# mako443/Text2Pos-CVPR2022

Hardware: AMD Instinct MI355X
Metric: cells+queries encoded/sec and top-k retrieval QPS, 256-pt cells, 12k-cell DB (higher is better)
Workload: dtype f16x3 (fp32 operands split hi+lo into fp16, 3 f16 MFMAs, fp32 accumulate; fp32-class error) for the encoders / f64 MFMA for the ranking

## Files before the change

include/t2p.h:

```cpp
#ifndef T2P_H
#define T2P_H
#include <stddef.h>
#include <stdint.h>

#ifdef __cplusplus
extern "C" {
#endif

#define T2P_ABI_VERSION 32
#define T2P_DEFAULT_CHUNK_OBJECTS 65000
#define T2P_MAX_CHUNK_OBJECTS 65535
#define T2P_TUNING_MASK 0xD
#define T2P_E_ARG (-1)
#define T2P_E_WORKSPACE (-2)
#define T2P_E_UNSUPPORTED (-3)

typedef void* t2p_stream_t;

int t2p_abi_version(void);
const char* t2p_last_error(void);

typedef struct t2p_cell_weights {
    const float* sa_w1[3];
    const float* sa_b1[3];
// ... 177 lines not shown
    const float* w_ih;
    const float* w_hh;
    const float* bias;
    const void* w_hh_x3;
    float w_hh_scale;
} t2p_text_weights;

size_t t2p_encode_text_workspace_bytes(int64_t batch, int32_t vocab, int32_t embed_dim);

int t2p_encode_text(const int32_t* tokens, const int32_t* lengths, int64_t batch, int32_t max_len, int32_t vocab,
                    int32_t embed_dim, const t2p_text_weights* w, float* out_raw, float* out, void* workspace,
                    size_t workspace_bytes, t2p_stream_t stream);

#define T2P_SIM_TOPK_MAX_K 1024
#define T2P_SIM_TOPK_REG_K 16
#define T2P_SIM_TOPK_TILE_BYTES ((size_t)256 << 20)
size_t t2p_sim_topk_workspace_bytes(int64_t nq, int64_t nc, int32_t k);
int t2p_sim_topk(const float* queries, const float* cells, int64_t nq, int64_t nc, int32_t dim, int32_t k,
                 int64_t index_offset, int64_t* out_idx, double* out_score, void* workspace, size_t workspace_bytes,
                 t2p_stream_t stream);
int t2p_sim_topk_grouped(const float* queries, const float* cells, const int32_t* query_group, const int32_t* cell_group,
                         int64_t nq, int64_t nc, int32_t dim, int32_t k, int64_t index_offset, int64_t* out_idx,
                         double* out_score, void* workspace, size_t workspace_bytes, t2p_stream_t stream);

void t2p_profile_enable(int on);
int t2p_profile_report(char* buf, size_t buf_bytes);
void t2p_profile_repeat(const char* scope, int32_t reps);

int t2p_lstm_train_forward(const float* gate_table, const float* w_hh_k, const int32_t* tokens, const int32_t* lengths,
                           int64_t batch, int32_t max_len, int32_t embed_dim, int32_t reverse, float* gates, float* cs, float* hs,
// ... 44 lines not shown
int t2p_sample_group(const float* xyz, int64_t n_obj, int32_t n_pts, const float* radius_host ,
                     uint8_t* const* fps_idx , uint8_t* const* nbr , uint8_t* const* cnt ,
                     t2p_stream_t stream);
int t2p_group_rows(const float* xyz, int64_t n_obj, int32_t n_pts, const float* radius_host , int32_t self_loops,
                   uint8_t* const* fps_idx , uint16_t* const* rows , uint16_t* const* n_rows ,
                   t2p_stream_t stream);
int t2p_group_rows_shared(const float* xyz, int64_t n_obj, int32_t n_pts, const float* radius_host , int32_t self_loops,
                          int32_t share_mask, uint8_t* const* fps_idx , uint16_t* const* rows ,
                          uint16_t* const* n_rows , t2p_stream_t stream);
int t2p_group_rows_built(const float* xyz, const float* rgb, int64_t n_obj, int32_t n_pts, const float* radius_host ,
                         int32_t self_loops, int32_t share_mask, uint8_t* const* fps_idx , uint16_t* const* rows ,
                         uint16_t* const* n_rows , t2p_stream_t stream);
int t2p_group_rows_pruned(const float* xyz, const float* rgb, int64_t n_obj, int32_t n_pts, const float* radius_host ,
                          int32_t self_loops, int32_t share_mask, uint8_t* const* fps_idx , uint16_t* const* rows ,
                          uint16_t* const* n_rows , t2p_stream_t stream);
int t2p_edge_counts(const uint16_t* rows, const uint16_t* n_rows, const int32_t* first_obj, int64_t n_obj, int32_t n_dense,
                    int32_t n_cent, int32_t self_loops, int32_t* counts, t2p_stream_t stream);
int t2p_edge_expand(const uint16_t* rows, const uint16_t* n_rows, const int32_t* first_obj, const int32_t* cent_ptr, int64_t n_obj,
                    int32_t n_dense, int32_t n_cent, int32_t self_loops, int32_t* src, int32_t* dst, t2p_stream_t stream);
int t2p_dedup_rows(const float* xyz, const float* rgb, int64_t n_obj, int32_t n_pts, uint16_t* rows, uint16_t* n_rows,
                   t2p_stream_t stream);
int t2p_knn(const float* x, int32_t dim, const int32_t* seg_ptr, int32_t n_seg, int32_t max_seg_rows, int32_t k,
            int32_t* out_idx, t2p_stream_t stream);
int t2p_gemm(const float* a, int32_t lda, const float* w, const float* bias, float* c, int32_t ldc, int32_t c0,
             int64_t m, int32_t k, int32_t n, int32_t relu, t2p_stream_t stream);
int t2p_gemm_residual(const float* a, int32_t lda, const float* w, const float* bias, float* c, int32_t ldc, int32_t c0,
                      int64_t m, int32_t k, int32_t n, int32_t relu, const float* resid, int32_t ldr, t2p_stream_t stream);
int t2p_gemm_x3(const float* a, int32_t lda, const void* wx, float scale, const float* bias, float* c, int32_t ldc, int32_t c0,
                int64_t m, int32_t k, int32_t n, int32_t relu, const float* resid, int32_t ldr, uint32_t* amax_in,
                t2p_stream_t stream);
// ... 15 lines not shown
```

profiles/topk_sweep.py:

```python
import argparse
import json
import os
import sys

import numpy as np
import torch

ROOT = os.path.dirname(os.path.dirname(os.path.abspath(__file__)))
sys.path.insert(0, ROOT)
import text2pos_amd as t2p
from text2pos_amd import ops


def timed(fn, steps, warmup, calls):
    ms = []
    for i in range(warmup + steps):
        e0, e1 = torch.cuda.Event(enable_timing=True), torch.cuda.Event(enable_timing=True)
        e0.record()
        for _ in range(calls):
            fn()
        e1.record()
        e1.synchronize()
        if i >= warmup:
            ms.append(e0.elapsed_time(e1) / calls)
# ... 6 lines not shown
        e0.record()
        for _ in range(calls):
            fn()
        e1.record()
        e1.synchronize()
        return e0.elapsed_time(e1) / calls
    a_ms, b_ms = [], []
    for i in range(warmup + steps):
        ta, tb = window(fn_a), window(fn_b)
        if i >= warmup:
            a_ms.append(ta)
            b_ms.append(tb)
    return float(np.median(a_ms)), float(np.median(b_ms)), [b / a for a, b in zip(a_ms, b_ms)]


def main():
    ap = argparse.ArgumentParser()
    ap.add_argument("--shapes", default="1000x12000,1250x100000")
    ap.add_argument("--ks", default="10,16,17,32,100,256,1024")
    ap.add_argument("--dim", type=int, default=256)
    ap.add_argument("--steps", type=int, default=9)
    ap.add_argument("--warmup", type=int, default=3)
    ap.add_argument("--calls", type=int, default=0, help="calls per timed window (0: 20 for the small shape, 3 above 10^8 scores)")
    ap.add_argument("--groups", type=int, default=0, help="also time the group-restricted call with this many group ids")
    ap.add_argument("--skip-torch", action="store_true", help="do not time torch's float64 GEMM + topk")
    a = ap.parse_args()
    assert torch.cuda.is_available(), "topk_sweep needs cuda:0: there is no CPU path to time"
    dev = torch.device("cuda:0")
    for shape in a.shapes.split(","):
        nq, nc = (int(x) for x in shape.split("x"))
        g = torch.Generator().manual_seed(nq * 31 + nc)
        c = torch.nn.functional.normalize(torch.randn(nc, a.dim, generator=g), dim=-1).to(dev)
        q = torch.nn.functional.normalize(torch.randn(nq, a.dim, generator=g), dim=-1).to(dev)
        calls = a.calls or (20 if nq * nc <= 10 ** 8 else 3)
        cd, qd = c.double(), q.double()
        if a.groups:
            cg = torch.randint(0, a.groups, (nc,), generator=g).to(torch.int32).to(dev)
            qg = torch.randint(0, a.groups, (nq,), generator=g).to(torch.int32).to(dev)
        for k in (int(x) for x in a.ks.split(",")):
            med, lo, hi = timed(lambda: t2p.retrieve_topk(c, q, k), a.steps, a.warmup, calls)
            t_med, t_lo, t_hi = (0.0, 0.0, 0.0) if a.skip_torch else timed(lambda: (qd @ cd.T).topk(k), a.steps, a.warmup, calls)
            grouped = {}
            if a.groups:
                u_ms, g_ms, ratios = timed_pairs(lambda: t2p.retrieve_topk(c, q, k),
# ... 33 lines not shown
```

text2pos-cvpr2022_amd/_lib.py:

```python
import ctypes as C
import os

import torch

_HERE = os.path.dirname(os.path.abspath(__file__))
LIB_PATH = os.environ.get("T2P_LIB") or os.path.join(_HERE, "libt2p_hip.so")
ABI_VERSION = 32

c_float_p = C.POINTER(C.c_float)
c_void = C.c_void_p


class CellWeights(C.Structure):
    _names = (["sa_w1", "sa_b1", "sa_w2", "sa_b2"], ["ga_w1", "ga_b1", "ga_w2", "ga_b2", "lin1_w", "lin1_b", "lin2_w",
              "lin2_b", "pn_w", "pn_b", "col_w1", "col_b1", "col_w2", "col_b2", "pos_w1", "pos_b1", "pos_w2", "pos_b2",
              "merge_w", "merge_b", "g_wp", "g_bp", "g_wq", "g_w2", "g_b2", "lin_w1", "lin_b1", "lin_w2", "lin_b2"])
    _fields_ = ([(n, c_void * 3) for n in _names[0]] + [(n, c_void) for n in _names[1]] +
                [("sa_w2_x3", c_void * 3), ("ga_w2_x3", c_void), ("sa_b2_x3", c_void * 3), ("sa_w2_scale", C.c_float * 3),
                 ("lin1_x3", c_void), ("lin2_x3", c_void), ("merge_x3", c_void), ("pn_x3", c_void), ("g_wp_x3", c_void),
                 ("g_wq_x3", c_void), ("lin1_scale", C.c_float), ("lin2_scale", C.c_float), ("merge_scale", C.c_float),
                 ("pn_scale", C.c_float), ("g_wp_scale", C.c_float), ("g_wq_scale", C.c_float),
                 ("sa_w1_x3", c_void * 3), ("ga_w1_x3", c_void),
                 ("class_embedding", c_void), ("color_embedding", c_void),
                 ("ga_w1_l1", C.c_float), ("ga_b1_absmax", C.c_float), ("sa_wp_l1", C.c_float * 3),
# ... 104 lines not shown
                                     C.c_int64, c_void, c_void, c_void, c_void, c_void, c_void, c_void]),
    "t2p_colsum": (C.c_int, [c_void, C.c_int64, C.c_int32, c_void, c_void]),
    "t2p_profile_enable": (None, [C.c_int]),
    "t2p_profile_report": (C.c_int, [C.c_char_p, C.c_size_t]),
    "t2p_profile_repeat": (None, [C.c_char_p, C.c_int32]),
    "t2p_sample_group": (C.c_int, [c_void, C.c_int64, C.c_int32, c_float_p, C.POINTER(c_void), C.POINTER(c_void),
                                   C.POINTER(c_void), c_void]),
    "t2p_group_rows": (C.c_int, [c_void, C.c_int64, C.c_int32, c_float_p, C.c_int32, C.POINTER(c_void), C.POINTER(c_void),
                                 C.POINTER(c_void), c_void]),
    "t2p_group_rows_shared": (C.c_int, [c_void, C.c_int64, C.c_int32, c_float_p, C.c_int32, C.c_int32, C.POINTER(c_void),
                                        C.POINTER(c_void), C.POINTER(c_void), c_void]),
    "t2p_group_rows_built": (C.c_int, [c_void, c_void, C.c_int64, C.c_int32, c_float_p, C.c_int32, C.c_int32, C.POINTER(c_void),
                                       C.POINTER(c_void), C.POINTER(c_void), c_void]),
    "t2p_group_rows_pruned": (C.c_int, [c_void, c_void, C.c_int64, C.c_int32, c_float_p, C.c_int32, C.c_int32, C.POINTER(c_void),
                                        C.POINTER(c_void), C.POINTER(c_void), c_void]),
    "t2p_edge_counts": (C.c_int, [c_void, c_void, c_void, C.c_int64, C.c_int32, C.c_int32, C.c_int32, c_void, c_void]),
    "t2p_edge_expand": (C.c_int, [c_void, c_void, c_void, c_void, C.c_int64, C.c_int32, C.c_int32, C.c_int32, c_void, c_void, c_void]),
    "t2p_dedup_rows": (C.c_int, [c_void, c_void, C.c_int64, C.c_int32, c_void, c_void, c_void]),
    "t2p_knn": (C.c_int, [c_void, C.c_int32, c_void, C.c_int32, C.c_int32, C.c_int32, c_void, c_void]),
    "t2p_gemm": (C.c_int, [c_void, C.c_int32, c_void, c_void, c_void, C.c_int32, C.c_int32, C.c_int64, C.c_int32,
                           C.c_int32, C.c_int32, c_void]),
    "t2p_rownorm": (C.c_int, [c_void, C.c_int64, C.c_int32, c_void, c_void]),
    "t2p_gemm_residual": (C.c_int, [c_void, C.c_int32, c_void, c_void, c_void, C.c_int32, C.c_int32, C.c_int64, C.c_int32,
                                    C.c_int32, C.c_int32, c_void, C.c_int32, c_void]),
    "t2p_gemm_x3": (C.c_int, [c_void, C.c_int32, c_void, C.c_float, c_void, c_void, C.c_int32, C.c_int32, C.c_int64, C.c_int32,
                              C.c_int32, C.c_int32, c_void, C.c_int32, c_void, c_void]),
    "t2p_gemm_skinny": (C.c_int, [c_void, C.c_int32, c_void, c_void, C.c_int32, C.c_int64, C.c_int32, C.c_int32, c_void]),
    "t2p_linear_wgrad_workspace_bytes": (C.c_size_t, [C.c_int64, C.c_int32, C.c_int32]),
    "t2p_linear_wgrad_f32": (C.c_int, [c_void, C.c_int32, c_void, C.c_int32, c_void, C.c_int32, c_void, C.c_int64, C.c_int32,
                                       C.c_int32, c_void, C.c_size_t, c_void]),
# ... 34 lines not shown
```

text2pos-cvpr2022_amd/csrc/api.hip:

```cpp
#include <stdarg.h>
#include <stdlib.h>
#include <math.h>
#include <string.h>

#include <mutex>
#include <set>
#include <utility>

#include "../../include/t2p.h"
#include "t2p_common.h"

namespace t2p {

static thread_local char g_err[512] = "";

void set_error(const char* fmt, ...) {
    va_list ap;
    va_start(ap, fmt);
    vsnprintf(g_err, sizeof(g_err), fmt, ap);
    va_end(ap);
}

int num_cus() {
    static int cached = 0;
// ... 374 lines not shown
    return launch_sim_topk(queries, cells, nq, nc, dim, k, index_offset, out_idx, out_score, workspace, workspace_bytes,
                           (hipStream_t)stream);
}

int t2p_sim_topk_grouped(const float* queries, const float* cells, const int32_t* query_group, const int32_t* cell_group,
                         int64_t nq, int64_t nc, int32_t dim, int32_t k, int64_t index_offset, int64_t* out_idx,
                         double* out_score, void* workspace, size_t workspace_bytes, t2p_stream_t stream) {
    T2P_CHECK_ARG(nq >= 0 && nc >= 0, "sim_topk_grouped: negative size");
    T2P_CHECK_ARG((queries != nullptr || nq == 0) && (cells != nullptr || nc == 0) &&
                      ((out_idx != nullptr && out_score != nullptr) || nq == 0 || k < 1),
                  "sim_topk_grouped: NULL argument");
    return launch_sim_topk_grouped(queries, cells, query_group, cell_group, nq, nc, dim, k, index_offset, out_idx, out_score,
                                   workspace, workspace_bytes, (hipStream_t)stream);
}

int t2p_edge_counts(const uint16_t* rows, const uint16_t* n_rows, const int32_t* first_obj, int64_t n_obj, int32_t n_dense,
                    int32_t n_cent, int32_t self_loops, int32_t* counts, t2p_stream_t stream) {
    T2P_CHECK_ARG(n_obj >= 0 && (n_obj == 0 || (rows && n_rows && first_obj && counts)), "edge_counts: NULL argument");
    return launch_edge_counts(rows, n_rows, first_obj, n_obj, n_dense, n_cent, self_loops, counts, (hipStream_t)stream);
}

int t2p_edge_expand(const uint16_t* rows, const uint16_t* n_rows, const int32_t* first_obj, const int32_t* cent_ptr, int64_t n_obj,
                    int32_t n_dense, int32_t n_cent, int32_t self_loops, int32_t* src, int32_t* dst, t2p_stream_t stream) {
    T2P_CHECK_ARG(n_obj >= 0 && (n_obj == 0 || (rows && n_rows && first_obj && cent_ptr)), "edge_expand: NULL argument");
    return launch_edge_expand(rows, n_rows, first_obj, cent_ptr, n_obj, n_dense, n_cent, self_loops, src, dst, (hipStream_t)stream);
}

int t2p_pack_objects(const float* raw_xyz, const float* raw_rgb, const int32_t* obj_ptr, const int32_t* sample_idx,
                     const float* rot_cos_sin, int64_t n_obj, int32_t n_pts, float* xyz, float* rgb, float* center, float* mean_rgb,
                     t2p_stream_t stream) {
// ... 105 lines not shown
```

text2pos-cvpr2022_amd/csrc/sim_topk.hip:

```cpp
#include "t2p_common.h"

namespace t2p {
namespace {

constexpr int KREG = 16;
constexpr int KCAP = KREG;
constexpr int KMAX = 1024;
constexpr int QB = 128;
constexpr int CB = 32;
typedef double f64x2 __attribute__((ext_vector_type(2)));
typedef int i32x4 __attribute__((ext_vector_type(4)));

struct Cand {
    double s;
    int i;
};
__device__ __forceinline__ bool better(double s, int i, double s2, int i2) { return s > s2 || (s == s2 && i < i2); }

__device__ __forceinline__ int d_row(int lane, int reg) { return (lane >> 4) + 4 * reg; }

__device__ __forceinline__ int tile_pos(int c) { return (c & ~15) | ((c & 3) << 2) | ((c >> 2) & 3); }

template <int DIM, bool GROUPED, class Epi>
__device__ __forceinline__ void sim_product_loop(const float* __restrict__ Q, const float* __restrict__ Cm, int64_t nq,
// ... 430 lines not shown
}

template <int DIM>
void launch_scores(dim3 grid, hipStream_t st, const float* Q, const float* Cm, const int32_t* qg, const int32_t* cg, int64_t nq,
                   int64_t nc, int cps, double* S, int64_t ld_s) {
    if (qg) hipLaunchKernelGGL((k_sim_scores<DIM, true>), grid, dim3(256), 0, st, Q, Cm, qg, cg, nq, nc, cps, S, ld_s);
    else hipLaunchKernelGGL((k_sim_scores<DIM, false>), grid, dim3(256), 0, st, Q, Cm, qg, cg, nq, nc, cps, S, ld_s);
}
template <int DIM>
void launch_partial(dim3 grid, hipStream_t st, const float* Q, const float* Cm, const int32_t* qg, const int32_t* cg, int64_t nq,
                    int64_t nc, int cps, double* ps, int* pi, int sp) {
    if (qg) hipLaunchKernelGGL((k_sim_partial<DIM, true>), grid, dim3(256), 0, st, Q, Cm, qg, cg, nq, nc, cps, ps, pi, sp);
    else hipLaunchKernelGGL((k_sim_partial<DIM, false>), grid, dim3(256), 0, st, Q, Cm, qg, cg, nq, nc, cps, ps, pi, sp);
}

int sim_topk_impl(const float* Q, const float* Cm, const int32_t* qg, const int32_t* cg, int64_t nq, int64_t nc, int dim, int k,
                  int64_t c_index_offset, int64_t* out_idx, double* out_score, void* ws, size_t ws_bytes, hipStream_t st);

}

size_t sim_topk_workspace_bytes(int64_t nq, int64_t nc, int k) {
    if (k > KREG) return (size_t)score_chunk(nq, nc) * score_ld(nc) * sizeof(double) + 256;
    const int sp = pick_splits(nq, nc);
    return (size_t)nq * sp * 4 * KCAP * (sizeof(double) + sizeof(int)) + 256;
}

int launch_sim_topk(const float* Q, const float* Cm, int64_t nq, int64_t nc, int dim, int k, int64_t c_index_offset,
                    int64_t* out_idx, double* out_score, void* ws, size_t ws_bytes, hipStream_t st) {
    return sim_topk_impl(Q, Cm, nullptr, nullptr, nq, nc, dim, k, c_index_offset, out_idx, out_score, ws, ws_bytes, st);
}

int launch_sim_topk_grouped(const float* Q, const float* Cm, const int32_t* query_group, const int32_t* cell_group, int64_t nq,
                            int64_t nc, int dim, int k, int64_t c_index_offset, int64_t* out_idx, double* out_score, void* ws,
                            size_t ws_bytes, hipStream_t st) {
    T2P_CHECK_ARG((query_group != nullptr || nq == 0) && (cell_group != nullptr || nc == 0), "sim_topk_grouped: NULL group array");
    return sim_topk_impl(Q, Cm, query_group, cell_group, nq, nc, dim, k, c_index_offset, out_idx, out_score, ws, ws_bytes, st);
}
// ... 2 lines not shown
int sim_topk_impl(const float* Q, const float* Cm, const int32_t* qg, const int32_t* cg, int64_t nq, int64_t nc, int dim, int k,
                  int64_t c_index_offset, int64_t* out_idx, double* out_score, void* ws, size_t ws_bytes, hipStream_t st) {
    T2P_CHECK_ARG(k >= 1 && k <= KMAX, "sim_topk: k=%d outside [1,%d]", k, KMAX);
    T2P_CHECK_ARG(dim == 256 || dim == 128 || dim == 384, "sim_topk: dim=%d not instantiated (128, 256, 384)", dim);
    T2P_CHECK_ARG(nc < 0x7fffffff, "sim_topk: nc too large");
    T2P_CHECK_ARG((((uintptr_t)Q) & 15) == 0 && (((uintptr_t)Cm) & 15) == 0, "sim_topk: Q and C must be 16-byte aligned");
    T2P_CHECK_ARG(k <= KREG || score_chunk(1, nc) > 0,
                  "sim_topk: k=%d > %d keeps one query's float64 scores (8 B x nc=%lld) in a workspace tile of at most %zu B: nc too large",
                  k, KREG, (long long)nc, kScoreTileBytes);
    if (nq == 0) return 0;
    const size_t need = sim_topk_workspace_bytes(nq, nc, k);
    if (ws_bytes < need || ws == nullptr) {
        set_error("sim_topk: workspace %zu B < required %zu B", ws_bytes, need);
        return T2P_E_WORKSPACE;
    }
    if (k > KREG) {
        T2P_CHECK_ARG((((uintptr_t)ws) & 15) == 0, "sim_topk: workspace must be 16-byte aligned");
        const int64_t chunk = score_chunk(nq, nc), ld_s = score_ld(nc);
        double* S = (double*)ws;
        for (int64_t qa = 0; qa < nq; qa += chunk) {
            const int64_t n = (nq - qa) < chunk ? (nq - qa) : chunk;
            if (nc > 0) {
                const int sp = pick_splits(n, nc);
                int cps = (int)((nc + sp - 1) / sp);
                cps = ((cps + CB - 1) / CB) * CB;
                const dim3 grid((unsigned)((n + QB - 1) / QB), (unsigned)sp);
                ProfScope ps_("sim_scores", st);
                const int32_t* qga = qg ? qg + qa : nullptr;
                if (dim == 256) launch_scores<256>(grid, st, Q + qa * dim, Cm, qga, cg, n, nc, cps, S, ld_s);
                else if (dim == 384) launch_scores<384>(grid, st, Q + qa * dim, Cm, qga, cg, n, nc, cps, S, ld_s);
                else launch_scores<128>(grid, st, Q + qa * dim, Cm, qga, cg, n, nc, cps, S, ld_s);
// ... 33 lines not shown
```

text2pos-cvpr2022_amd/csrc/small_kernels.hip:

```cpp
#include "t2p_common.h"

namespace t2p {
namespace {

__global__ __launch_bounds__(256) void k_rownorm(const float* __restrict__ in, int ld_in, int64_t n_rows, int dim,
                                                 float* __restrict__ out, int ld_out, int col0) {
    const int lane = threadIdx.x & 63;
    int64_t row = (int64_t)blockIdx.x * 4 + (threadIdx.x >> 6);
    if (row >= n_rows) return;
    const float* x = in + row * ld_in;
    float ss = 0.f;
    for (int i = lane; i < dim; i += 64) ss = fmaf(x[i], x[i], ss);
#pragma unroll
    for (int off = 32; off >= 1; off >>= 1) ss += __shfl_xor(ss, off, 64);
    float nrm = sqrtf(ss);
    float den = nrm > 1e-12f ? nrm : 1e-12f;
    float* y = out + row * ld_out + col0;
    for (int i = lane; i < dim; i += 64) y[i] = x[i] / den;
}

__global__ __launch_bounds__(256) void k_gather_rownorm(const float* __restrict__ table, const int32_t* __restrict__ idx,
                                                        int64_t n_rows, int dim, float* __restrict__ out, int ld_out,
                                                        int col0) {
    const int lane = threadIdx.x & 63;
// ... 147 lines not shown
        for (int off = 32; off >= 1; off >>= 1) v += __shfl_xor(v, off, 64);
        if ((tid & 63) == 0) ss[tid >> 6][r] = v;
    }
    __syncthreads();
#pragma unroll
    for (int j = 0; j < 2; j++) {
        const int c = tid + 256 * j;
        if (c >= D) break;
#pragma unroll
        for (int r = 0; r < kMlp3Rows; r++) {
            if (row0 + r >= n_rows) break;
            const float nrm = sqrtf((ss[0][r] + ss[1][r]) + (ss[2][r] + ss[3][r]));
            out[(row0 + r) * ld_out + col0 + c] = o[j][r] / (nrm > 1e-12f ? nrm : 1e-12f);
        }
    }
}

__device__ __forceinline__ uint64_t pack_mix64(uint64_t x) {
    x += 0x9E3779B97F4A7C15ull;
    x = (x ^ (x >> 30)) * 0xBF58476D1CE4E5B9ull;
    x = (x ^ (x >> 27)) * 0x94D049BB133111EBull;
    return x ^ (x >> 31);
}

__device__ __forceinline__ void aten_column_sums(const float* __restrict__ pts, int n_pts, int lane, float& sx, float& sy, float& sz) {
    float part = 0.f;
    if (lane < 12) {
        const int c = lane >> 2, k = lane & 3;
        const int size_ilp = n_pts >> 2;
        float acc[4] = {0.f, 0.f, 0.f, 0.f};
// ... 340 lines not shown
}

int launch_segmax(const float* in, int dim, const int32_t* seg_ptr, int n_seg, float* out, int mean, hipStream_t st) {
    if (n_seg == 0) return 0;
    ProfScope ps_("segpool", st);
    hipLaunchKernelGGL(k_segpool, dim3(n_seg), dim3(256), 0, st, in, dim, seg_ptr, n_seg, out, mean);
    T2P_CHECK_LAUNCH("segpool");
    return 0;
}

int launch_mlp3_norm(const float* in3, int64_t n_rows, const float* w1, const float* b1, const float* w2,
                     const float* b2, int D, float* out, int ld_out, int col0, hipStream_t st) {
    T2P_CHECK_ARG(D % 64 == 0 && D <= 512, "mlp3_norm: D=%d must be a multiple of 64, <= 512", D);
    if (n_rows == 0) return 0;
    ProfScope ps_("mlp3_norm", st);
    if (n_rows >= 16384)
        hipLaunchKernelGGL(k_mlp3_norm<32>, dim3((unsigned)((n_rows + 31) / 32)), dim3(256), 0, st, in3, n_rows, w1, b1, w2, b2, D, out, ld_out,
                           col0);
    else
        hipLaunchKernelGGL(k_mlp3_norm<8>, dim3((unsigned)((n_rows + 7) / 8)), dim3(256), 0, st, in3, n_rows, w1, b1, w2, b2, D, out, ld_out,
                           col0);
    T2P_CHECK_LAUNCH("mlp3_norm");
    return 0;
}

int launch_pack_objects(const float* raw_xyz, const float* raw_rgb, const int32_t* obj_ptr, const int32_t* sample_idx,
                        const float* rot, int64_t n_obj, int n_pts, float* xyz, float* rgb, float* center, float* mean_rgb,
                        hipStream_t st) {
    T2P_CHECK_ARG(n_pts <= 1024, "pack_objects: n_pts=%d > 1024 (the sampled points of an object are staged in LDS)", n_pts);
    if (n_obj == 0) return 0;
    ProfScope ps_("pack_objects", st);
    hipLaunchKernelGGL(k_pack_objects, dim3((unsigned)((n_obj + 3) / 4)), dim3(256), (size_t)4 * n_pts * 3 * sizeof(float), st, raw_xyz,
                       raw_rgb, obj_ptr, sample_idx, rot, n_obj, n_pts, xyz, rgb, center, mean_rgb);
    T2P_CHECK_LAUNCH("pack_objects");
// ... 88 lines not shown
```

text2pos-cvpr2022_amd/csrc/t2p_common.h:

```cpp
#pragma once
#include <hip/hip_runtime.h>
#include <stdint.h>
#include <stdio.h>

namespace t2p {

void set_error(const char* fmt, ...);

#define T2P_E_ARG (-1)
#define T2P_E_WORKSPACE (-2)
#define T2P_E_UNSUPPORTED (-3)

#define T2P_CHECK_ARG(cond, ...)                  \
    do {                                          \
        if (!(cond)) {                            \
            ::t2p::set_error(__VA_ARGS__);        \
            return T2P_E_ARG;                     \
        }                                         \
    } while (0)

#define T2P_CHECK_LAUNCH(name)                                                   \
    do {                                                                         \
        hipError_t e__ = hipGetLastError();                                      \
        if (e__ != hipSuccess) {                                                 \
// ... 253 lines not shown
    const float* pos_src;
    int ld_pos, pos_col0;
    const float* feat_src;
    const float* w1;
    const float* b1;
    int n_dense, n_cent;
    int64_t n_obj;
    int32_t* prefix_ws;
    int32_t* bounds_ws;
    int balanced;
    uint32_t* amax_out;
    int out_rows;
};
int launch_ws_sa(int H, int C, const SaParams& p, hipStream_t st);
int launch_sa_balance(const SaParams& p, int tile_rows, int n_wg, hipStream_t st);
constexpr int kSaTailCode = 64;
bool sa_rows_selected(int H, int C, const SaParams& p);
int launch_sa_rows(int H, int C, const SaParams& p, hipStream_t st);
int sa_rows_launch_shape(int64_t n_obj, int* tile_rows, int* n_wg);
bool sa_points_selected(int H, int C, const SaParams& p);
int launch_sa_points(int H, int C, const SaParams& p, hipStream_t st);
int sa_points_launch_shape(int64_t n_obj, int* tile_rows, int* n_wg);
bool sa3_selected(int H, int C, const SaParams& p);
int launch_sa3(const SaParams& p, hipStream_t st);
int sa3_launch_shape(int64_t n_obj, int* tile_rows, int* n_wg);
inline bool sa_shares_tail_rows(int l, int H, int C, const SaParams& p, int n_pts, int tuning) {
    return l == 1 && n_pts == 256 && !(tuning & 4) && p.n_dense == 128 && p.n_cent == 64 && sa_rows_selected(H, C, p);
}
int launch_sa_balance_levels(const SaParams p[3], const int H[3], const int C[3], hipStream_t st);

// ... 47 lines not shown
```

text2pos-cvpr2022_amd/csrc/ws_sa.hip:

```cpp
#include <type_traits>

#include "t2p_common.h"

namespace t2p {
namespace {

constexpr int kSub = 512;
constexpr int NT = 512;

template <int K, int N, int WN, int RT, bool X3>
struct SaCfg {
    static constexpr int WM = 8 / WN;
    static constexpr int NTW = N / (32 * WN);
    static constexpr int TR = WM * RT * 32;
    static constexpr int KS = K / 2;
    static constexpr int S16 = K / 16;
    static constexpr int WPLANES = X3 ? 2 : 1;
    static constexpr int WSTEPS = X3 ? S16 : KS;
    static constexpr int LD = X3 ? K + 8 : K + 4;
    static constexpr int PLANE = TR * LD;
    static constexpr int ACC_INTS = 8192 + N;
    static constexpr int F4_PER_ROW = K / 4;
    static constexpr int ITERS = TR * F4_PER_ROW / NT;
    static_assert(TR * F4_PER_ROW % NT == 0, "staging must divide evenly over the workgroup");
    static_assert(ITERS == 2 || ITERS == 4, "metadata vector is 4 or 8 bytes");
    static constexpr size_t lds_bytes() {
        return (size_t)2 * PLANE * 4 + (size_t)2 * ACC_INTS * 4 + 2 * TR + kSub * 2 + kSub * 4;
    }
};

__device__ __forceinline__ void balance_body(const uint16_t* __restrict__ n_rows, int n, int tile_rows, int n_wg,
                                             int32_t* __restrict__ prefix, int32_t* __restrict__ bounds) {
    __shared__ int part[1024];
    const int tid = threadIdx.x;
    const int per = (n + 1023) / 1024;
    const int lo = tid * per, hi = (lo + per) < n ? (lo + per) : n;
    int s = 0;
    for (int i = lo; i < hi; i++) s += ((int)n_rows[i] + tile_rows - 1) / tile_rows;
    part[tid] = s;
    __syncthreads();
    for (int off = 1; off < 1024; off <<= 1) {
        int v = tid >= off ? part[tid - off] : 0;
        __syncthreads();
        part[tid] += v;
        __syncthreads();
    }
    int run = part[tid] - s;
    for (int i = lo; i < hi; i++) {
        prefix[i] = run;
        run += ((int)n_rows[i] + tile_rows - 1) / tile_rows;
    }
    if (tid == 1023) prefix[n] = part[1023];
    __syncthreads();
    const int total = part[1023];
    for (int b = tid; b <= n_wg; b += 1024) {
        const long long target = ((long long)b * total) / n_wg;
        int l = 0, r = n;
        while (l < r) {
            const int m = (l + r) >> 1;
            if (prefix[m] < target) l = m + 1; else r = m;
        }
        bounds[b] = b == n_wg ? n : l;
    }
}

__global__ __launch_bounds__(1024) void k_balance(const uint16_t* __restrict__ n_rows, int n, int tile_rows, int n_wg,
                                                  int32_t* __restrict__ prefix, int32_t* __restrict__ bounds) {
    balance_body(n_rows, n, tile_rows, n_wg, prefix, bounds);
}

struct BalanceJobs {
    const uint16_t* n_rows[3];
    int32_t* prefix[3];
    int32_t* bounds[3];
    int tile_rows[3], n_wg[3];
    int n;
};
__global__ __launch_bounds__(1024) void k_balance_levels(BalanceJobs j) {
    const int l = blockIdx.x;
    balance_body(j.n_rows[l], j.n, j.tile_rows[l], j.n_wg[l], j.prefix[l], j.bounds[l]);
}

struct BatchIt {
    int gi;
    int r0;
    int n;
};

template <int K, int N, int WN, int RT, bool X3>
__global__ __launch_bounds__(NT, 2) void k_sa_stream(SaParams p) {
    using C = SaCfg<K, N, WN, RT, X3>;
    using TileT = std::conditional_t<X3, _Float16, float>;
    using WReg = std::conditional_t<X3, half8, float>;
// ... 246 lines not shown
            if (valid(it_d)) write_tile((t + 1) & 1, meta_d);
            fix_meta(it_m, meta_m);
            meta_d = meta_m;
            it_c = it_d;
            it_d = it_m;
            it_m = advance(it_m);
            __syncthreads();
        }
        if (flush_g >= 0) flush(flush_g, flush_buf);
    }
    if constexpr (X3) guard_publish_exact(p.amax_out, gmax);
}

}

int launch_sa_balance(const SaParams& p, int tile_rows, int n_wg, hipStream_t st) {
    ProfScope ps_("sa_balance", st);
    hipLaunchKernelGGL(k_balance, dim3(1), dim3(1024), 0, st, p.n_rows, (int)p.n_obj, tile_rows, n_wg, p.prefix_ws,
                       p.bounds_ws);
    T2P_CHECK_LAUNCH("sa_balance");
    return 0;
}

namespace {

#define SA_STREAM_CASES(X) X(32, 64, 2, 2) X(128, 128, 4, 1) X(256, 256, 8, 1)

int sa_stream_shape(int H, int Cout, bool x3, int64_t n_obj, int* tile_rows, int* n_wg) {
    int n = num_cus();
    if (n > 1024) n = 1024;
    if (n > n_obj) n = (int)n_obj;
    *n_wg = n;
#define SA_CASE(K_, N_, WN_, RT_)                           \
    if (H == K_ && Cout == N_) {                            \
        *tile_rows = SaCfg<K_, N_, WN_, RT_, false>::TR;    \
        return 0;                                           \
// ... 69 lines not shown
}

}

int launch_sa_balance_levels(const SaParams p[3], const int H[3], const int C[3], hipStream_t st) {
    if (p[0].n_obj <= 0) return 0;
    BalanceJobs j;
    j.n = (int)p[0].n_obj;
    for (int l = 0; l < 3; l++) {
        j.n_rows[l] = p[l].n_rows;
        j.prefix[l] = p[l].prefix_ws;
        j.bounds[l] = p[l].bounds_ws;
        T2P_TRY(sa_launch_shape(H[l], C[l], p[l], p[l].n_obj, &j.tile_rows[l], &j.n_wg[l]));
    }
    ProfScope ps_("sa_balance", st);
    hipLaunchKernelGGL(k_balance_levels, dim3(3), dim3(1024), 0, st, j);
    T2P_CHECK_LAUNCH("sa_balance");
    return 0;
}

int launch_ws_sa(int H, int Cout, const SaParams& p, hipStream_t st) {
    T2P_CHECK_ARG((((uintptr_t)p.A | (uintptr_t)p.Bc) & 15) == 0, "ws_sa: tables must be 16-byte aligned");
    if (p.W_x3 != nullptr) T2P_CHECK_ARG(((uintptr_t)p.W_x3 & 15) == 0, "ws_sa: packed f16x3 weights must be 16-byte aligned");
    switch (sa_pick(H, Cout, p)) {
        case SA_ROWS: return launch_sa_rows(H, Cout, p, st);
        case SA_POINTS: return launch_sa_points(H, Cout, p, st);
        case SA_3: return launch_sa3(p, st);
        case SA_X3:
        case SA_FP32: return launch_sa_stream(H, Cout, p, st);
        case SA_NONE: break;
    }
// ... 5 lines not shown
```

text2pos-cvpr2022_amd/ops.py:

```python
import ctypes as C
import os
from typing import Dict, Optional

import numpy as np
import torch

from . import _lib as L

_workspaces: Dict[tuple, torch.Tensor] = {}


def _stream(device) -> C.c_void_p:
    return C.c_void_p(torch.cuda.current_stream(device).cuda_stream)


def _ptr(t: Optional[torch.Tensor]) -> C.c_void_p:
    return C.c_void_p(0 if t is None else t.data_ptr())


def _need(t: torch.Tensor, name: str, dtype, ndim=None, device=None):
    if not isinstance(t, torch.Tensor):
        raise RuntimeError(f"{name}: expected a torch.Tensor, got {type(t).__name__}")
    if not t.is_cuda:
        raise RuntimeError(f"{name}: must live on the GPU (got device {t.device}); there is no CPU path")
# ... 171 lines not shown
        L.check(L.lib().t2p_edge_counts(_ptr(rows[l]), _ptr(n_rows[l]), _ptr(first_obj), n_obj, nd, nc,
                                        int(bool(self_loops)), _ptr(counts), st), "t2p_edge_counts")
        cp = torch.zeros((n_obj * nc + 1,), dtype=torch.int32, device=dev)
        torch.cumsum(counts, 0, dtype=torch.int32, out=cp[1:])
        cent_ptrs.append(cp)
    totals = torch.stack([cp[-1] for cp in cent_ptrs]).cpu().tolist()
    out = []
    for l, (nd, nc) in enumerate(levels):
        e = int(totals[l])
        src = torch.empty((e,), dtype=torch.int32, device=dev)
        dst = torch.empty((e,), dtype=torch.int32, device=dev)
        L.check(L.lib().t2p_edge_expand(_ptr(rows[l]), _ptr(n_rows[l]), _ptr(first_obj), _ptr(cent_ptrs[l]), n_obj, nd, nc,
                                        int(bool(self_loops)), _ptr(src), _ptr(dst), st), "t2p_edge_expand")
        out.append(dict(fps_idx=t["fps_idx"][l], src=src, dst=dst, cent_ptr=cent_ptrs[l], n_dense=nd, n_cent=nc))
    return out


def group_rows(xyz: torch.Tensor, radius=(0.2, 0.3, 0.4), self_loops: bool = True, share_mask: int = 0):
    _need(xyz, "xyz", torch.float32, 3)
    dev = xyz.device
    n_obj, n_pts, three = xyz.shape
    if three != 3:
        raise RuntimeError(f"xyz: last dimension must be 3, got {three}")
    out, arr = _level_tables(n_obj, n_pts, dev, ("fps_idx", "rows", "n_rows"))
    L.check(L.lib().t2p_group_rows_shared(_ptr(xyz), n_obj, n_pts, _radius(radius), int(bool(self_loops)), int(share_mask),
                                          arr["fps_idx"], arr["rows"], arr["n_rows"], _stream(dev)), "t2p_group_rows_shared")
    return out


def group_rows_built(xyz: torch.Tensor, rgb: torch.Tensor, radius=(0.2, 0.3, 0.4), self_loops: bool = True, share_mask: int = 0,
# ... 970 lines not shown
```

Measured before the change: 160,600.

## Rework SA balance scan, add row-wave mlp3 kernel, route large top-k to score tile

Three changes land together. The single-block balance kernel now does a vectorized warp-shuffle prefix scan with a coarse shared-memory index for the bound search, replacing the strided serial scan and the global binary search. A new k_mlp3_rows kernel handles large row counts with one row per lane and weights broadcast by readlane, replacing k_mlp3_norm<32>. Top-k with k <= 16 is sent to the score-tile path when the query-cell pair count is large. An API wrapper for the balance kernel and a sweep option are also added; the mlp3 kernel's register pressure is the main risk.

```diff
diff --git a/include/t2p.h b/include/t2p.h
--- a/include/t2p.h
+++ b/include/t2p.h
@@ -215,6 +215,7 @@
 
 #define T2P_SIM_TOPK_MAX_K 1024
 #define T2P_SIM_TOPK_REG_K 16
+#define T2P_SIM_TOPK_TILE_MIN_PAIRS 256000
 #define T2P_SIM_TOPK_TILE_BYTES ((size_t)256 << 20)
 size_t t2p_sim_topk_workspace_bytes(int64_t nq, int64_t nc, int32_t k);
 int t2p_sim_topk(const float* queries, const float* cells, int64_t nq, int64_t nc, int32_t dim, int32_t k,
@@ -289,6 +290,8 @@
 int t2p_group_rows_pruned(const float* xyz, const float* rgb, int64_t n_obj, int32_t n_pts, const float* radius_host ,
                           int32_t self_loops, int32_t share_mask, uint8_t* const* fps_idx , uint16_t* const* rows ,
                           uint16_t* const* n_rows , t2p_stream_t stream);
+int t2p_sa_balance(const uint16_t* n_rows, int32_t n, int32_t tile_rows, int32_t n_wg, int32_t* prefix ,
+                   int32_t* bounds , t2p_stream_t stream);
 int t2p_edge_counts(const uint16_t* rows, const uint16_t* n_rows, const int32_t* first_obj, int64_t n_obj, int32_t n_dense,
                     int32_t n_cent, int32_t self_loops, int32_t* counts, t2p_stream_t stream);
 int t2p_edge_expand(const uint16_t* rows, const uint16_t* n_rows, const int32_t* first_obj, const int32_t* cent_ptr, int64_t n_obj,
diff --git a/profiles/topk_sweep.py b/profiles/topk_sweep.py
--- a/profiles/topk_sweep.py
+++ b/profiles/topk_sweep.py
@@ -44,6 +44,9 @@
     return float(np.median(a_ms)), float(np.median(b_ms)), [b / a for a, b in zip(a_ms, b_ms)]
 
 
+ROUTE_SHAPES = ",".join(f"{nq}x{nc}" for nq in (64, 130, 256, 1000, 1250) for nc in (1000, 4000, 12000, 100000))
+
+
 def main():
     ap = argparse.ArgumentParser()
     ap.add_argument("--shapes", default="1000x12000,1250x100000")
@@ -57,7 +60,7 @@
     a = ap.parse_args()
     assert torch.cuda.is_available(), "topk_sweep needs cuda:0: there is no CPU path to time"
     dev = torch.device("cuda:0")
-    for shape in a.shapes.split(","):
+    for shape in (ROUTE_SHAPES if a.shapes == "route" else a.shapes).split(","):
         nq, nc = (int(x) for x in shape.split("x"))
         g = torch.Generator().manual_seed(nq * 31 + nc)
         c = torch.nn.functional.normalize(torch.randn(nc, a.dim, generator=g), dim=-1).to(dev)
diff --git a/text2pos-cvpr2022_amd/_lib.py b/text2pos-cvpr2022_amd/_lib.py
--- a/text2pos-cvpr2022_amd/_lib.py
+++ b/text2pos-cvpr2022_amd/_lib.py
@@ -142,6 +142,7 @@
                                        C.POINTER(c_void), C.POINTER(c_void), c_void]),
     "t2p_group_rows_pruned": (C.c_int, [c_void, c_void, C.c_int64, C.c_int32, c_float_p, C.c_int32, C.c_int32, C.POINTER(c_void),
                                         C.POINTER(c_void), C.POINTER(c_void), c_void]),
+    "t2p_sa_balance": (C.c_int, [c_void, C.c_int32, C.c_int32, C.c_int32, c_void, c_void, c_void]),
     "t2p_edge_counts": (C.c_int, [c_void, c_void, c_void, C.c_int64, C.c_int32, C.c_int32, C.c_int32, c_void, c_void]),
     "t2p_edge_expand": (C.c_int, [c_void, c_void, c_void, c_void, C.c_int64, C.c_int32, C.c_int32, C.c_int32, c_void, c_void, c_void]),
     "t2p_dedup_rows": (C.c_int, [c_void, c_void, C.c_int64, C.c_int32, c_void, c_void, c_void]),
diff --git a/text2pos-cvpr2022_amd/csrc/api.hip b/text2pos-cvpr2022_amd/csrc/api.hip
--- a/text2pos-cvpr2022_amd/csrc/api.hip
+++ b/text2pos-cvpr2022_amd/csrc/api.hip
@@ -412,6 +412,14 @@
                                    workspace, workspace_bytes, (hipStream_t)stream);
 }
 
+int t2p_sa_balance(const uint16_t* n_rows, int32_t n, int32_t tile_rows, int32_t n_wg, int32_t* prefix, int32_t* bounds,
+                   t2p_stream_t stream) {
+    T2P_CHECK_ARG(n >= 0 && tile_rows >= 1 && n_wg >= 1, "sa_balance: n=%d tile_rows=%d n_wg=%d (n >= 0, tile_rows >= 1, n_wg >= 1)", n,
+                  tile_rows, n_wg);
+    T2P_CHECK_ARG((n_rows != nullptr || n == 0) && prefix != nullptr && bounds != nullptr, "sa_balance: NULL argument");
+    return launch_sa_balance_arrays(n_rows, n, tile_rows, n_wg, prefix, bounds, (hipStream_t)stream);
+}
+
 int t2p_edge_counts(const uint16_t* rows, const uint16_t* n_rows, const int32_t* first_obj, int64_t n_obj, int32_t n_dense,
                     int32_t n_cent, int32_t self_loops, int32_t* counts, t2p_stream_t stream) {
     T2P_CHECK_ARG(n_obj >= 0 && (n_obj == 0 || (rows && n_rows && first_obj && counts)), "edge_counts: NULL argument");
diff --git a/text2pos-cvpr2022_amd/csrc/sim_topk.hip b/text2pos-cvpr2022_amd/csrc/sim_topk.hip
--- a/text2pos-cvpr2022_amd/csrc/sim_topk.hip
+++ b/text2pos-cvpr2022_amd/csrc/sim_topk.hip
@@ -6,6 +6,10 @@
 constexpr int KREG = 16;
 constexpr int KCAP = KREG;
 constexpr int KMAX = 1024;
+#ifndef T2P_SIM_TILE_MIN_PAIRS
+#define T2P_SIM_TILE_MIN_PAIRS 256000
+#endif
+constexpr int64_t kTileMinPairs = T2P_SIM_TILE_MIN_PAIRS;
 constexpr int QB = 128;
 constexpr int CB = 32;
 typedef double f64x2 __attribute__((ext_vector_type(2)));
@@ -468,13 +472,19 @@
     else hipLaunchKernelGGL((k_sim_partial<DIM, false>), grid, dim3(256), 0, st, Q, Cm, qg, cg, nq, nc, cps, ps, pi, sp);
 }
 
+bool use_score_tile(int64_t nq, int64_t nc, int k) {
+    if (k > KREG) return true;
+    const bool large = nq > 0 && nc > 0 && (nq >= kTileMinPairs || nc >= (kTileMinPairs + nq - 1) / nq);
+    return large && score_chunk(1, nc) > 0;
+}
+
 int sim_topk_impl(const float* Q, const float* Cm, const int32_t* qg, const int32_t* cg, int64_t nq, int64_t nc, int dim, int k,
                   int64_t c_index_offset, int64_t* out_idx, double* out_score, void* ws, size_t ws_bytes, hipStream_t st);
 
 }
 
 size_t sim_topk_workspace_bytes(int64_t nq, int64_t nc, int k) {
-    if (k > KREG) return (size_t)score_chunk(nq, nc) * score_ld(nc) * sizeof(double) + 256;
+    if (use_score_tile(nq, nc, k)) return (size_t)score_chunk(nq, nc) * score_ld(nc) * sizeof(double) + 256;
     const int sp = pick_splits(nq, nc);
     return (size_t)nq * sp * 4 * KCAP * (sizeof(double) + sizeof(int)) + 256;
 }
@@ -507,7 +517,7 @@
         set_error("sim_topk: workspace %zu B < required %zu B", ws_bytes, need);
         return T2P_E_WORKSPACE;
     }
-    if (k > KREG) {
+    if (use_score_tile(nq, nc, k)) {
         T2P_CHECK_ARG((((uintptr_t)ws) & 15) == 0, "sim_topk: workspace must be 16-byte aligned");
         const int64_t chunk = score_chunk(nq, nc), ld_s = score_ld(nc);
         double* S = (double*)ws;
diff --git a/text2pos-cvpr2022_amd/csrc/small_kernels.hip b/text2pos-cvpr2022_amd/csrc/small_kernels.hip
--- a/text2pos-cvpr2022_amd/csrc/small_kernels.hip
+++ b/text2pos-cvpr2022_amd/csrc/small_kernels.hip
@@ -185,6 +185,134 @@
             out[(row0 + r) * ld_out + col0 + c] = o[j][r] / (nrm > 1e-12f ? nrm : 1e-12f);
         }
     }
+}
+
+template <int K0>
+__device__ __forceinline__ void mlp3_k8(const float (&hid)[64], const float* __restrict__ wl, int D, float (&o)[64]) {
+    float wv[8];
+#pragma unroll
+    for (int i = 0; i < 8; i++) wv[i] = wl[(K0 + i) * D];
+#pragma unroll
+    for (int i = 0; i < 8; i++) {
+#pragma unroll
+        for (int c0 = 0; c0 < 64; c0 += 8) {
+            float w[8];
+#pragma unroll
+            for (int e = 0; e < 8; e++) w[e] = __builtin_bit_cast(float, __builtin_amdgcn_readlane(__builtin_bit_cast(int, wv[i]), c0 + e));
+#pragma unroll
+            for (int e = 0; e < 8; e++) o[c0 + e] = fmaf(hid[K0 + i], w[e], o[c0 + e]);
+        }
+    }
+}
+
+__device__ __forceinline__ void mlp3_slice(const float (&hid)[64], const float* __restrict__ w2, const float* __restrict__ b2, int D,
+                                           int cbase, int lane, float (&o)[64]) {
+#pragma unroll
+    for (int c = 0; c < 64; c++) o[c] = b2[cbase + c];
+    const float* wl = w2 + cbase + lane;
+    mlp3_k8<0>(hid, wl, D, o);
+    mlp3_k8<8>(hid, wl, D, o);
+    mlp3_k8<16>(hid, wl, D, o);
+    mlp3_k8<24>(hid, wl, D, o);
+    mlp3_k8<32>(hid, wl, D, o);
+    mlp3_k8<40>(hid, wl, D, o);
+    mlp3_k8<48>(hid, wl, D, o);
+    mlp3_k8<56>(hid, wl, D, o);
+#pragma unroll
+    for (int c = 0; c < 64; c++) o[c] = fmaxf(o[c], 0.f);
+}
+
+__device__ __forceinline__ void mlp3_store(const float (&o)[64], float den, bool have, float (*tile)[36], int lane, int64_t row0,
+                                           int64_t n_rows, float* __restrict__ out, int ld_out, int c_first, bool vec_out) {
+#pragma unroll
+    for (int half = 0; half < 2; half++) {
+        if (have) {
+#pragma unroll
+            for (int q = 0; q < 8; q++) {
+                f32x4 t;
+#pragma unroll
+                for (int e = 0; e < 4; e++) t[e] = o[half * 32 + q * 4 + e] / den;
+                *(f32x4*)&tile[lane][q * 4] = t;
+            }
+        }
+        __syncthreads();
+        if (have) {
+#pragma unroll
+            for (int it = 0; it < 8; it++) {
+                const int r = it * 8 + (lane >> 3), c4 = (lane & 7) * 4;
+                const f32x4 t = *(const f32x4*)&tile[r][c4];
+                if (row0 + r < n_rows) {
+                    float* dst = out + (row0 + r) * ld_out + c_first + half * 32 + c4;
+                    if (vec_out) *(f32x4*)dst = t;
+                    else {
+#pragma unroll
+                        for (int e = 0; e < 4; e++) dst[e] = t[e];
+                    }
+                }
+            }
+        }
+        __syncthreads();
+    }
+}
+
+template <int NJ>
+__global__ __launch_bounds__(256) void k_mlp3_rows(const float* __restrict__ in3, int64_t n_rows,
+                                                   const float* __restrict__ w1, const float* __restrict__ b1,
+                                                   const float* __restrict__ w2, const float* __restrict__ b2, int D,
+                                                   float* __restrict__ out, int ld_out, int col0) {
+    constexpr int TLD = 36;
+    __shared__ __attribute__((aligned(16))) float tile[4][64][TLD];
+    __shared__ float ss[4][64];
+    const int lane = threadIdx.x & 63;
+    const int wave = __builtin_amdgcn_readfirstlane(threadIdx.x >> 6);
+    const int n_wave = blockDim.x >> 6;
+    const int64_t row0 = (int64_t)blockIdx.x * 64;
+    const int64_t row = row0 + lane;
+    float x0 = 0.f, x1 = 0.f, x2 = 0.f;
+    if (row < n_rows) {
+        x0 = in3[row * 3];
+        x1 = in3[row * 3 + 1];
+        x2 = in3[row * 3 + 2];
+    }
+    float hid[64];
+#pragma unroll
+    for (int u = 0; u < 64; u++) {
+        float a = b1[u];
+        a = fmaf(x0, w1[u], a);
+        a = fmaf(x1, w1[64 + u], a);
+        a = fmaf(x2, w1[128 + u], a);
+        hid[u] = fmaxf(a, 0.f);
+    }
+    const int cbase = 64 * wave;
+    const bool have1 = NJ > 1 && 256 + cbase < D;
+    float o0[64];
+    [[maybe_unused]] float o1[NJ > 1 ? 64 : 1];
+    mlp3_slice(hid, w2, b2, D, cbase, lane, o0);
+    if constexpr (NJ > 1) mlp3_slice(hid, w2, b2, D, have1 ? 256 + cbase : cbase, lane, o1);
+    {
+        float v[64];
+#pragma unroll
+        for (int l = 0; l < 64; l++) {
+            v[l] = fmaf(o0[l], o0[l], 0.f);
+            if constexpr (NJ > 1) {
+                if (have1) v[l] = fmaf(o1[l], o1[l], v[l]);
+            }
+        }
+#pragma unroll
+        for (int off = 32; off >= 1; off >>= 1) {
+#pragma unroll
+            for (int l = 0; l < off; l++) v[l] = v[l] + v[l + off];
+        }
+        ss[wave][lane] = v[0];
+    }
+    __syncthreads();
+    const float p0 = ss[0][lane], p1 = n_wave > 1 ? ss[1][lane] : 0.f, p2 = n_wave > 2 ? ss[2][lane] : 0.f,
+                p3 = n_wave > 3 ? ss[3][lane] : 0.f;
+    const float nrm = sqrtf((p0 + p1) + (p2 + p3));
+    const float den = nrm > 1e-12f ? nrm : 1e-12f;
+    const bool vec_out = ((((uintptr_t)out) & 15) == 0) && (ld_out & 3) == 0 && (col0 & 3) == 0;
+    mlp3_store(o0, den, true, tile[wave], lane, row0, n_rows, out, ld_out, col0 + cbase, vec_out);
+    if constexpr (NJ > 1) mlp3_store(o1, den, have1, tile[wave], lane, row0, n_rows, out, ld_out, col0 + 256 + cbase, vec_out);
 }
 
 __device__ __forceinline__ uint64_t pack_mix64(uint64_t x) {
@@ -555,10 +683,11 @@
     T2P_CHECK_ARG(D % 64 == 0 && D <= 512, "mlp3_norm: D=%d must be a multiple of 64, <= 512", D);
     if (n_rows == 0) return 0;
     ProfScope ps_("mlp3_norm", st);
-    if (n_rows >= 16384)
-        hipLaunchKernelGGL(k_mlp3_norm<32>, dim3((unsigned)((n_rows + 31) / 32)), dim3(256), 0, st, in3, n_rows, w1, b1, w2, b2, D, out, ld_out,
-                           col0);
-    else
+    if (n_rows >= 16384) {
+        const dim3 grid((unsigned)((n_rows + 63) / 64)), block(64 * (D >= 256 ? 4 : D / 64));
+        if (D > 256) hipLaunchKernelGGL(k_mlp3_rows<2>, grid, block, 0, st, in3, n_rows, w1, b1, w2, b2, D, out, ld_out, col0);
+        else hipLaunchKernelGGL(k_mlp3_rows<1>, grid, block, 0, st, in3, n_rows, w1, b1, w2, b2, D, out, ld_out, col0);
+    } else
         hipLaunchKernelGGL(k_mlp3_norm<8>, dim3((unsigned)((n_rows + 7) / 8)), dim3(256), 0, st, in3, n_rows, w1, b1, w2, b2, D, out, ld_out,
                            col0);
     T2P_CHECK_LAUNCH("mlp3_norm");
diff --git a/text2pos-cvpr2022_amd/csrc/t2p_common.h b/text2pos-cvpr2022_amd/csrc/t2p_common.h
--- a/text2pos-cvpr2022_amd/csrc/t2p_common.h
+++ b/text2pos-cvpr2022_amd/csrc/t2p_common.h
@@ -291,6 +291,7 @@
 };
 int launch_ws_sa(int H, int C, const SaParams& p, hipStream_t st);
 int launch_sa_balance(const SaParams& p, int tile_rows, int n_wg, hipStream_t st);
+int launch_sa_balance_arrays(const uint16_t* n_rows, int n, int tile_rows, int n_wg, int32_t* prefix, int32_t* bounds, hipStream_t st);
 constexpr int kSaTailCode = 64;
 bool sa_rows_selected(int H, int C, const SaParams& p);
 int launch_sa_rows(int H, int C, const SaParams& p, hipStream_t st);
diff --git a/text2pos-cvpr2022_amd/csrc/ws_sa.hip b/text2pos-cvpr2022_amd/csrc/ws_sa.hip
--- a/text2pos-cvpr2022_amd/csrc/ws_sa.hip
+++ b/text2pos-cvpr2022_amd/csrc/ws_sa.hip
@@ -29,42 +29,111 @@
     }
 };
 
+constexpr int kBalT = 1024;
+constexpr int kBalCoarse = 8192;
+
 __device__ __forceinline__ void balance_body(const uint16_t* __restrict__ n_rows, int n, int tile_rows, int n_wg,
                                              int32_t* __restrict__ prefix, int32_t* __restrict__ bounds) {
-    __shared__ int part[1024];
-    const int tid = threadIdx.x;
-    const int per = (n + 1023) / 1024;
-    const int lo = tid * per, hi = (lo + per) < n ? (lo + per) : n;
-    int s = 0;
-    for (int i = lo; i < hi; i++) s += ((int)n_rows[i] + tile_rows - 1) / tile_rows;
-    part[tid] = s;
+    __shared__ int coarse[kBalCoarse + 1];
+    __shared__ int wtot[2][kBalT / 64];
+    const int tid = threadIdx.x, lane = tid & 63, wave = tid >> 6;
+    int sh = 3;
+    while ((n >> sh) > kBalCoarse) sh++;
+    const bool vec_in = (((uintptr_t)n_rows) & 15) == 0, vec_out = (((uintptr_t)prefix) & 15) == 0;
+    const unsigned tr = (unsigned)tile_rows;
+
+    typedef uint16_t u16x8 __attribute__((ext_vector_type(8)));
+    typedef int i32x4 __attribute__((ext_vector_type(4)));
+    auto load8 = [&](int i0) -> u16x8 {
+        u16x8 v = {0, 0, 0, 0, 0, 0, 0, 0};
+        if (i0 + 8 <= n && vec_in) v = *(const u16x8*)(n_rows + i0);
+        else {
+#pragma unroll
+            for (int e = 0; e < 8; e++)
+                if (i0 + e < n) v[e] = n_rows[i0 + e];
+        }
+        return v;
+    };
+
+    int carry = 0;
+    u16x8 cur = load8(tid * 8);
+    for (int base = 0, it = 0; base < n; base += kBalT * 8, it++) {
+        const int i0 = base + tid * 8;
+        u16x8 nxt = {0, 0, 0, 0, 0, 0, 0, 0};
+        if (base + kBalT * 8 < n) nxt = load8(i0 + kBalT * 8);
+        int t[8], s = 0;
+#pragma unroll
+        for (int e = 0; e < 8; e++) {
+            t[e] = (int)(((unsigned)cur[e] + tr - 1) / tr);
+            s += t[e];
+        }
+        int inc = s;
+#pragma unroll
+        for (int o = 1; o < 64; o <<= 1) {
+            const int up = __shfl_up(inc, o, 64);
+            if (lane >= o) inc += up;
+        }
+        if (lane == 63) wtot[it & 1][wave] = inc;
+        __syncthreads();
+        int before = 0, all = 0;
+#pragma unroll
+        for (int w = 0; w < kBalT / 64; w++) {
+            const int v = wtot[it & 1][w];
+            before += w < wave ? v : 0;
+            all += v;
+        }
+        int run = carry + before + inc - s;
+        carry += all;
+        if (i0 < n && (i0 & ((1 << sh) - 1)) == 0) coarse[i0 >> sh] = run;
+        int p[8];
+#pragma unroll
+        for (int e = 0; e < 8; e++) {
+            p[e] = run;
+            run += t[e];
+        }
+        if (i0 + 8 <= n && vec_out) {
+            *(i32x4*)(prefix + i0) = i32x4{p[0], p[1], p[2], p[3]};
+            *(i32x4*)(prefix + i0 + 4) = i32x4{p[4], p[5], p[6], p[7]};
+        } else {
+#pragma unroll
+            for (int e = 0; e < 8; e++)
+                if (i0 + e < n) prefix[i0 + e] = p[e];
+        }
+        cur = nxt;
+    }
+    const int total = carry;
+    if (tid == 0) {
+        prefix[n] = total;
+        if ((n & ((1 << sh) - 1)) == 0) coarse[n >> sh] = total;
+    }
     __syncthreads();
-    for (int off = 1; off < 1024; off <<= 1) {
-        int v = tid >= off ? part[tid - off] : 0;
-        __syncthreads();
-        part[tid] += v;
-        __syncthreads();
-    }
-    int run = part[tid] - s;
-    for (int i = lo; i < hi; i++) {
-        prefix[i] = run;
-        run += ((int)n_rows[i] + tile_rows - 1) / tile_rows;
-    }
-    if (tid == 1023) prefix[n] = part[1023];
-    __syncthreads();
-    const int total = part[1023];
-    for (int b = tid; b <= n_wg; b += 1024) {
+    const int n_coarse = (n >> sh) + 1;
+    for (int b = tid; b <= n_wg; b += kBalT) {
         const long long target = ((long long)b * total) / n_wg;
-        int l = 0, r = n;
+        int l = 0, r = n_coarse;
         while (l < r) {
             const int m = (l + r) >> 1;
-            if (prefix[m] < target) l = m + 1; else r = m;
-        }
-        bounds[b] = b == n_wg ? n : l;
-    }
-}
-
-__global__ __launch_bounds__(1024) void k_balance(const uint16_t* __restrict__ n_rows, int n, int tile_rows, int n_wg,
+            if (coarse[m] < target) l = m + 1; else r = m;
+        }
+        int ans = 0;
+        if (l > 0) {
+            const int lo = ((l - 1) << sh) + 1;
+            const int hi = l < n_coarse ? (l << sh) : n;
+            int cnt = 0;
+            for (int x0 = lo; x0 < hi; x0 += 8) {
+                int v[8];
+#pragma unroll
+                for (int e = 0; e < 8; e++) v[e] = prefix[(x0 + e) < hi ? (x0 + e) : hi];
+#pragma unroll
+                for (int e = 0; e < 8; e++) cnt += ((x0 + e) < hi && v[e] < target) ? 1 : 0;
+            }
+            ans = lo + cnt;
+        }
+        bounds[b] = b == n_wg ? n : ans;
+    }
+}
+
+__global__ __launch_bounds__(kBalT) void k_balance(const uint16_t* __restrict__ n_rows, int n, int tile_rows, int n_wg,
                                                   int32_t* __restrict__ prefix, int32_t* __restrict__ bounds) {
     balance_body(n_rows, n, tile_rows, n_wg, prefix, bounds);
 }
@@ -76,7 +145,7 @@
     int tile_rows[3], n_wg[3];
     int n;
 };
-__global__ __launch_bounds__(1024) void k_balance_levels(BalanceJobs j) {
+__global__ __launch_bounds__(kBalT) void k_balance_levels(BalanceJobs j) {
     const int l = blockIdx.x;
     balance_body(j.n_rows[l], j.n, j.tile_rows[l], j.n_wg[l], j.prefix[l], j.bounds[l]);
 }
@@ -353,12 +422,15 @@
 
 }
 
-int launch_sa_balance(const SaParams& p, int tile_rows, int n_wg, hipStream_t st) {
+int launch_sa_balance_arrays(const uint16_t* n_rows, int n, int tile_rows, int n_wg, int32_t* prefix, int32_t* bounds, hipStream_t st) {
     ProfScope ps_("sa_balance", st);
-    hipLaunchKernelGGL(k_balance, dim3(1), dim3(1024), 0, st, p.n_rows, (int)p.n_obj, tile_rows, n_wg, p.prefix_ws,
-                       p.bounds_ws);
+    hipLaunchKernelGGL(k_balance, dim3(1), dim3(kBalT), 0, st, n_rows, n, tile_rows, n_wg, prefix, bounds);
     T2P_CHECK_LAUNCH("sa_balance");
     return 0;
+}
+
+int launch_sa_balance(const SaParams& p, int tile_rows, int n_wg, hipStream_t st) {
+    return launch_sa_balance_arrays(p.n_rows, (int)p.n_obj, tile_rows, n_wg, p.prefix_ws, p.bounds_ws, st);
 }
 
 namespace {
@@ -458,7 +530,7 @@
         T2P_TRY(sa_launch_shape(H[l], C[l], p[l], p[l].n_obj, &j.tile_rows[l], &j.n_wg[l]));
     }
     ProfScope ps_("sa_balance", st);
-    hipLaunchKernelGGL(k_balance_levels, dim3(3), dim3(1024), 0, st, j);
+    hipLaunchKernelGGL(k_balance_levels, dim3(3), dim3(kBalT), 0, st, j);
     T2P_CHECK_LAUNCH("sa_balance");
     return 0;
 }
diff --git a/text2pos-cvpr2022_amd/ops.py b/text2pos-cvpr2022_amd/ops.py
--- a/text2pos-cvpr2022_amd/ops.py
+++ b/text2pos-cvpr2022_amd/ops.py
@@ -209,6 +209,16 @@
                                         int(bool(self_loops)), _ptr(src), _ptr(dst), st), "t2p_edge_expand")
         out.append(dict(fps_idx=t["fps_idx"][l], src=src, dst=dst, cent_ptr=cent_ptrs[l], n_dense=nd, n_cent=nc))
     return out
+
+
+def sa_balance(n_rows: torch.Tensor, tile_rows: int, n_wg: int):
+    _need(n_rows, "n_rows", torch.int16, 1)
+    dev, n = n_rows.device, n_rows.shape[0]
+    prefix = torch.empty((n + 1,), dtype=torch.int32, device=dev)
+    bounds = torch.empty((int(n_wg) + 1,), dtype=torch.int32, device=dev)
+    L.check(L.lib().t2p_sa_balance(_ptr(n_rows), n, int(tile_rows), int(n_wg), _ptr(prefix), _ptr(bounds), _stream(dev)),
+            "t2p_sa_balance")
+    return prefix, bounds
 
 
 def group_rows(xyz: torch.Tensor, radius=(0.2, 0.3, 0.4), self_loops: bool = True, share_mask: int = 0):
```

New measurement: 162,200 (median of 6 runs). 1.01x the previous value.
